# zhaoyuhsin/Edge-Guided-Near-Eye-Image-Analysis-for-Head-Mounted-Displays

Measured on AMD Instinct MI355X. Metric: eye-frames/sec (320x240): inference edge+seg (value), +fit, exact fp32, and train fwd+bwd at 1 MI355X, higher is better.
Workload: dtype f32 tensors; inference products split into f16 hi/lo pairs (3 f16 MFMAs per product, 22-bit significand), f32 accumulate (`exact_fp32`: every product on the f32 MFMA); `train`: bf16 storage, f32 accumulate, f32 master weights (and an f32-storage leg)

## Files before the change

edge-guided-near-eye-image-analysis-for-head-mounted-displays_amd/csrc/common.h:

```cpp
#pragma once
#include <hip/hip_runtime.h>
#include <cstdarg>
#include <cstdio>
#include <mutex>
#include <unordered_map>
#include "../../include/egne_hip.h"

static __device__ __attribute__((aligned(256), used)) float egne_zero_page[64] = {0};

typedef __bf16 egne_bf16;
typedef float egne_f32x4 __attribute__((ext_vector_type(4)));
typedef __bf16 egne_bf16x4 __attribute__((ext_vector_type(4)));
typedef __bf16 egne_bf16x8 __attribute__((ext_vector_type(8)));

__device__ __forceinline__ egne_f32x4 ld4(const float* p) { return *(const egne_f32x4*)p; }
__device__ __forceinline__ egne_f32x4 ld4(const egne_bf16* p) { return __builtin_convertvector(*(const egne_bf16x4*)p, egne_f32x4); }
__device__ __forceinline__ void st4(float* p, egne_f32x4 v) { *(egne_f32x4*)p = v; }
__device__ __forceinline__ void st4(egne_bf16* p, egne_f32x4 v) { *(egne_bf16x4*)p = __builtin_convertvector(v, egne_bf16x4); }
__device__ __forceinline__ float ld1(const float* p) { return *p; }
__device__ __forceinline__ float ld1(const egne_bf16* p) { return (float)*p; }
__device__ __forceinline__ void st1(float* p, float v) { *p = v; }
__device__ __forceinline__ void st1(egne_bf16* p, float v) { *p = (egne_bf16)v; }
template <typename T> struct egne_vt { static constexpr int N = 4; };
template <> struct egne_vt<egne_bf16> { static constexpr int N = 8; };
template <int N> struct egne_fv { float v[N]; };
__device__ __forceinline__ egne_fv<4> ldv(const float* p) {
  const egne_f32x4 t = *(const egne_f32x4*)p;
  return egne_fv<4>{{t[0], t[1], t[2], t[3]}};
}
__device__ __forceinline__ egne_fv<8> ldv(const egne_bf16* p) {
  typedef unsigned u4_ __attribute__((ext_vector_type(4)));
  const u4_ w = *(const u4_*)p;
  egne_fv<8> r;
#pragma unroll
  for (int i = 0; i < 4; ++i) {
    r.v[2 * i] = __builtin_bit_cast(float, w[i] << 16);
    r.v[2 * i + 1] = __builtin_bit_cast(float, w[i] & 0xffff0000u);
  }
  return r;
}
__device__ __forceinline__ void stv(float* p, const egne_fv<4>& a) { *(egne_f32x4*)p = egne_f32x4{a.v[0], a.v[1], a.v[2], a.v[3]}; }
__device__ __forceinline__ void stv(egne_bf16* p, const egne_fv<8>& a) {
  const egne_f32x4 lo = {a.v[0], a.v[1], a.v[2], a.v[3]}, hi = {a.v[4], a.v[5], a.v[6], a.v[7]};
  const egne_bf16x4 l = __builtin_convertvector(lo, egne_bf16x4), h = __builtin_convertvector(hi, egne_bf16x4);
  *(egne_bf16x8*)p = egne_bf16x8{l[0], l[1], l[2], l[3], h[0], h[1], h[2], h[3]};
}
typedef unsigned egne_u32x4 __attribute__((ext_vector_type(4)));
template <typename T> __device__ __forceinline__ egne_u32x4 ldraw(const T* p) { return *(const egne_u32x4*)p; }
__device__ __forceinline__ egne_fv<4> unpackv(const float*, egne_u32x4 w) {
  return egne_fv<4>{{__builtin_bit_cast(float, w[0]), __builtin_bit_cast(float, w[1]), __builtin_bit_cast(float, w[2]), __builtin_bit_cast(float, w[3])}};
}
__device__ __forceinline__ egne_fv<8> unpackv(const egne_bf16*, egne_u32x4 w) {
  egne_fv<8> r;
#pragma unroll
  for (int i = 0; i < 4; ++i) {
    r.v[2 * i] = __builtin_bit_cast(float, w[i] << 16);
    r.v[2 * i + 1] = __builtin_bit_cast(float, w[i] & 0xffff0000u);
  }
  return r;
}
template <int N> __device__ __forceinline__ egne_fv<N> ldf(const float* p) {
  egne_fv<N> r;
#pragma unroll
  for (int i = 0; i < N; i += 4) { const egne_f32x4 t = *(const egne_f32x4*)(p + i); r.v[i] = t[0]; r.v[i + 1] = t[1]; r.v[i + 2] = t[2]; r.v[i + 3] = t[3]; }
  return r;
}
template <int N> __device__ __forceinline__ egne_fv<N> fv_fill(float x) {
  egne_fv<N> r;
#pragma unroll
  for (int i = 0; i < N; ++i) r.v[i] = x;
  return r;
}
template <typename T> __device__ __forceinline__ const T* zero_page() { return (const T*)egne_zero_page; }

#ifdef EGNE_NO_OVF_CHECK
__device__ __forceinline__ bool egne_nonfinite(float) { return false; }
__device__ __forceinline__ bool egne_nonfinite64(double) { return false; }
#else
__device__ __forceinline__ bool egne_nonfinite(float v) { return __builtin_amdgcn_classf(v, 0x207); }
__device__ __forceinline__ bool egne_nonfinite64(double v) { return !__builtin_isfinite(v); }
#endif
__device__ __forceinline__ bool egne_ovf_row(int y, int H) { return y % 3 == 1 || y == H - 1; }
__device__ __forceinline__ void egne_ovf_commit(bool bad, unsigned* flag) {
  if (flag && bad) atomicOr(flag, 1u);
}

namespace egne {

char* err_buf();

inline int fail(int code, const char* fmt, ...) {
  va_list ap;
  va_start(ap, fmt);
  vsnprintf(err_buf(), 512, fmt, ap);
  va_end(ap);
  return code;
}

inline bool fp32_storage(const egne_conv_desc& d) {
  for (int i = 0; i < d.nseg && i < EGNE_MAXSEG; ++i)
    if (d.seg[i].presplit != 0) return false;
  return d.out_split == 0;
}

inline int check_launch(const char* what) {
  hipError_t e = hipGetLastError();
  if (e != hipSuccess) return fail(EGNE_ERR_LAUNCH, "%s: %s", what, hipGetErrorString(e));
  return EGNE_OK;
}

inline bool raise_lds(const void* kern, size_t bytes) {
  static std::mutex mu;
  static std::unordered_map<const void*, size_t> have;
  std::lock_guard<std::mutex> g(mu);
  auto it = have.find(kern);
  if (it != have.end() && it->second >= bytes) return true;
  if (hipFuncSetAttribute(kern, hipFuncAttributeMaxDynamicSharedMemorySize, (int)bytes) != hipSuccess) {
    (void)hipGetLastError();
    return false;
  }
  have[kern] = bytes;
  return true;
}

#define EGNE_REQUIRE(cond, ...) \
  do { if (!(cond)) return ::egne::fail(EGNE_ERR_ARG, __VA_ARGS__); } while (0)

bool halo3_supported(const egne_conv_desc& d);
int halo3_launch(const egne_conv_desc& d, hipStream_t st);

bool wgrad_halo_supported(const egne_conv_desc& d, long long gzs);
int wgrad_halo_splits(const egne_conv_desc& d);
int wgrad_halo_launch(const egne_conv_desc& d, const float* gz, long long gzs, int gzo, float* ws, hipStream_t st);
int wgrad_halo_f16_launch(const egne_conv_desc& d, const float* gz, long long gzs, int gzo, const unsigned* gz_dyn, float* ws, hipStream_t st);

bool wgrad3x3_bf16_supported(const egne_conv_desc& d, long long gzs);
int wgrad3x3_bf16_splits(const egne_conv_desc& d);
int wgrad3x3_bf16_launch(const egne_conv_desc& d, const egne_bf16* gz, long long gzs, int gzo, float* ws, hipStream_t st);
bool wgrad1x1_bf16_supported(const egne_conv_desc& d, long long gzs);
int wgrad1x1_bf16_splits(const egne_conv_desc& d);
int wgrad1x1_bf16_launch(const egne_conv_desc& d, const egne_bf16* gz, long long gzs, int gzo, float* ws, hipStream_t st);

int msdil_ps_launch(const egne_conv_desc& d, const void* fhi, const void* flo, float a_scale, float w_scale, const float* score_w,
                    const float* score_c, float* s0, float* s1, int accumulate, hipStream_t st);

bool msdil1_wanted(const egne_conv_desc& d);
int msdil1_launch(const egne_conv_desc& d, const void* fhi, float a_scale, float w_scale, const float* score_w, const float* score_c,
                  float* s0, float* s1, int accumulate, hipStream_t st);

inline int cdiv(long long a, long long b) { return (int)((a + b - 1) / b); }

}
```

edge-guided-near-eye-image-analysis-for-head-mounted-displays_amd/csrc/msblock_dil_ps_f16.hip:

```cpp
#include "common.h"
#include <type_traits>

typedef float f32x4 __attribute__((ext_vector_type(4)));
typedef _Float16 h8 __attribute__((ext_vector_type(8)));
typedef unsigned u32x4 __attribute__((ext_vector_type(4)));
typedef __attribute__((address_space(3))) void* lds_ptr;

namespace {
__device__ int g_pdbg = 0;
__device__ unsigned long long g_pstamps[256 * 8 * 4];

constexpr int TW = 32, TH = 8;
constexpr int D0 = 4, D1 = 8, D2 = 12, DMAX = 12;
constexpr int SWMAX = TW + 2 * DMAX, NPXMAX = TH * SWMAX;
constexpr int PLANE = NPXMAX * 32 + 32;
constexpr int BUFH = 2 * PLANE;
constexpr int WBUFH = 12 * 512;
constexpr int NS = 9;
constexpr unsigned OOB = 0x80000000u;

__device__ __forceinline__ __amdgpu_buffer_rsrc_t make_rsrc(const void* base, unsigned bytes) {
  return __builtin_amdgcn_make_buffer_rsrc(const_cast<void*>(base), 0, (int)bytes, 0x00020000);
}

__device__ __forceinline__ void lds_barrier() {
  asm volatile("s_waitcnt lgkmcnt(0)" ::: "memory");
  __builtin_amdgcn_s_barrier();
  asm volatile("" ::: "memory");
}

constexpr int dil_of(int g) { return g == 0 ? D0 : (g == 1 ? D1 : D2); }
constexpr int ni_of(int g) { return TH * (TW + 2 * dil_of(g)) * 8 / 512; }

template <bool XIN, int NP = 3>
__global__ __launch_bounds__(512)
void msdil_ps_kernel(const egne_conv_desc p, const _Float16* __restrict__ fhi, const _Float16* __restrict__ flo, float inv_a, float out_scale,
                     int tiles_x, int tiles_y, int ntiles, int cols, const float* __restrict__ score_w, const float* __restrict__ score_c,
                     float* __restrict__ s0, float* __restrict__ s1, int accumulate) {
  extern __shared__ __attribute__((aligned(16))) _Float16 ldsh[];
  _Float16* const lw = ldsh + 2 * BUFH;
  float* const lconst = (float*)(lw + 3 * WBUFH);
  int* const lrel = (int*)(lconst + 162);

  const int dbg = g_pdbg;
  unsigned long long t_work = 0, t_wait = 0, t_last = __builtin_amdgcn_s_memtime();
  auto stamp = [&](unsigned long long& accum) {
    if (dbg & 64) {
      asm volatile("s_waitcnt lgkmcnt(0)" ::: "memory");
      const unsigned long long t = __builtin_amdgcn_s_memtime();
      accum += t - t_last; t_last = t;
    }
  };
  const int tid = threadIdx.x, lane = tid & 63;
  const int wave = __builtin_amdgcn_readfirstlane(tid >> 6);
  const int l15 = lane & 15, kg = lane >> 4;
  const int H = p.H, W = p.W;
  const egne_seg sg = p.seg[0];

  const int per = gridDim.x >> 3;
  auto tile_at = [&](int i) { return (gridDim.x & 7) ? (int)blockIdx.x + i * (int)gridDim.x : ((i * 8 + ((int)blockIdx.x & 7)) * per + ((int)blockIdx.x >> 3)); };
  struct Tile { int b, y0, x0; };
  auto decode = [&](int t) {
    Tile r;
    const int ntx = cols == 0 ? tiles_x : (cols == 1 ? tiles_x - 2 : 2);
    const int tq = t % ntx; t /= ntx;
    const int tx = cols == 0 ? tq : (cols == 1 ? tq + 1 : tq * (tiles_x - 1));
    const int ty = t % tiles_y; t /= tiles_y;
    r.b = t; r.y0 = ty * TH; r.x0 = tx * TW;
    return r;
  };
  int nmine = 0;
  while (tile_at(nmine) < ntiles) ++nmine;
  if (tid < 160) {
    const int r = tid >> 5, c = tid & 31;
    lconst[tid] = r < 3 ? (p.bias ? p.bias[r * p.CoutP + c] : 0.f) : (score_w ? score_w[(r - 3) * 32 + c] : 0.f);
  } else if (tid < 162) {
    lconst[tid] = score_c ? score_c[tid - 160] : 0.f;
  }

  const int piece = tid & 7, pg = tid >> 3;
  constexpr int NI0 = ni_of(0), NI1 = ni_of(1), NI2 = ni_of(2);
  u32x4 st0[NI0], st1[NI1], st2[NI2];
  auto stbuf = [&](auto gc) -> u32x4* { constexpr int Gq = decltype(gc)::value; if constexpr (Gq == 0) return st0; else if constexpr (Gq == 1) return st1; else return st2; };
  constexpr int RB1 = NI0, RB2 = NI0 + NI1;
  if constexpr (XIN) {
    for (int e = tid; e < (NI0 + NI1 + NI2) * 64; e += 512) {
      const int row = e >> 6, pgq = e & 63;
      const int g = row < RB1 ? 0 : (row < RB2 ? 1 : 2), I = row - (g == 0 ? 0 : (g == 1 ? RB1 : RB2));
      const int d = g == 0 ? D0 : (g == 1 ? D1 : D2), SW = TW + 2 * d;
      const int px = pgq + 64 * I;
      const int rr = px / SW, cc = px - rr * SW;
      lrel[e] = ((rr * W + cc - d) * (int)sg.pix_stride + sg.ch_off) * 4;
    }
  }
  const int lofs = (piece >> 2) * PLANE + pg * 32 + (((piece & 3) ^ ((pg >> 1) & 3)) << 3);
  const unsigned wbytes = 3u * 9u * 2u * 1024u;
  const __amdgpu_buffer_rsrc_t rwh = make_rsrc(fhi, wbytes), rwl = make_rsrc(flo, wbytes);

  auto dma_weights = [&](auto sc) {
    constexpr int S = decltype(sc)::value, g = S % 3, ky = S / 3;
    char* wb = (char*)(lw + g * WBUFH);
#pragma unroll
    for (int t = 0; t < 2; ++t) {
      const int j = t == 0 ? wave : 8 + (wave & 3), f = j >> 1;
      const int o = ((g * 9 + ky * 3 + (f >> 1)) * 2 + (f & 1)) * 1024;
      __builtin_amdgcn_raw_ptr_buffer_load_lds((j & 1) ? rwl : rwh, (lds_ptr)(wb + j * 1024), 16, lane * 16, o, 0, 0);
    }
  };
  auto issue_strip = [&](const Tile& tl, bool on, auto sc) {
    constexpr int S = decltype(sc)::value, g = S % 3, ky = S / 3, d = dil_of(g), SW = TW + 2 * d;
    const __amdgpu_buffer_rsrc_t r = make_rsrc(sg.ptr + (long long)tl.b * H * W * sg.pix_stride, (unsigned)H * W * (unsigned)sg.pix_stride * 4u);
    int pq = pg;
    asm volatile("" : "+v"(pq));
#pragma unroll
    for (int I = 0; I < ni_of(g); ++I) {
      int off;
      if constexpr (XIN) {
        const int sbase = ((tl.y0 + (ky - 1) * d) * W + tl.x0) * (int)sg.pix_stride * 4 + piece * 16;
        off = lrel[((g == 0 ? 0 : (g == 1 ? RB1 : RB2)) + I) * 64 + pq] + sbase;
      } else {
        const int px = pq + 64 * I;
        const int rr = px / SW, cc = px - rr * SW;
        const int y = tl.y0 + (ky - 1) * d + rr, x = tl.x0 - d + cc;
        off = ((y * W + x) * (int)sg.pix_stride + sg.ch_off + piece * 4) * 4;
        off = ((unsigned)x < (unsigned)W && (unsigned)y < (unsigned)H) ? off : (int)OOB;
      }
      stbuf(std::integral_constant<int, g>{})[I] = __builtin_amdgcn_raw_buffer_load_b128(r, (on && !(dbg & 1) && (NP == 3 || piece < 4)) ? off : (int)OOB, 0, 0);
    }
  };
  auto write_strip = [&](int q, auto sc) {
    constexpr int S = decltype(sc)::value, g = S % 3;
    _Float16* buf = ldsh + (q & 1) * BUFH;
    if (!(dbg & 2)) {
#pragma unroll
      for (int I = 0; I < ni_of(g); ++I) *(u32x4*)&buf[lofs + 32 * 64 * I] = stbuf(std::integral_constant<int, g>{})[I];
    }
  };

  const int wl = (kg >> 1) * 1024 + ((kg & 1) * 32 + l15) * 8;
  f32x4 acc[3][2][2];
  h8 resh[2], resl[2];
  auto compute_strip = [&](int q, auto sc) {
    constexpr int S = decltype(sc)::value, g = S % 3, ky = S / 3, d = dil_of(g), SW = TW + 2 * d;
    const _Float16* Shi = ldsh + (q & 1) * BUFH;
    const _Float16* Slo = Shi + PLANE;
    const _Float16* wb = lw + g * WBUFH + wl;
    if constexpr (ky == 0) {
#pragma unroll
      for (int a = 0; a < 4; ++a) (&acc[g][0][0])[a] = (f32x4)(0.f);
    }
    h8 wh[2], wo[2], ah[2][2], al[2][2];
    auto fetch_w = [&](auto kc) {
      constexpr int KX = decltype(kc)::value;
#pragma unroll
      for (int nh = 0; nh < 2; ++nh) {
        wh[nh] = *(const h8*)&wb[KX * 2048 + nh * 128];
        if constexpr (NP == 3) wo[nh] = *(const h8*)&wb[KX * 2048 + 512 + nh * 128];
      }
    };
    auto fetch = [&](auto kc) {
      constexpr int KX = decltype(kc)::value, Bq = KX & 1;
#pragma unroll
      for (int ph = 0; ph < 2; ++ph) {
        const int qq = wave * SW + ph * 16 + l15 + KX * d;
        const int o = qq * 32 + ((kg ^ ((qq >> 1) & 3)) << 3);
        ah[Bq][ph] = *(const h8*)&Shi[o];
        if constexpr (NP == 3 || (S == 3 && KX == 1)) al[Bq][ph] = *(const h8*)&Slo[o];
      }
    };
    fetch(std::integral_constant<int, 0>{});
    [&]<int... Ks>(std::integer_sequence<int, Ks...>) {
      (([&] {
        constexpr int kx = Ks, Bq = kx & 1;
        fetch_w(std::integral_constant<int, kx>{});
        if constexpr (kx + 1 < 3) fetch(std::integral_constant<int, kx + 1>{});
        if constexpr (S == 3 && kx == 1) { resh[0] = ah[1][0]; resh[1] = ah[1][1]; resl[0] = al[1][0]; resl[1] = al[1][1]; }
        __builtin_amdgcn_sched_barrier(0);
        if constexpr (NP == 3) {
#pragma unroll
        for (int ph = 0; ph < 2; ++ph)
#pragma unroll
          for (int nh = 0; nh < 2; ++nh) acc[g][ph][nh] = __builtin_amdgcn_mfma_f32_16x16x32_f16(wh[nh], al[Bq][ph], acc[g][ph][nh], 0, 0, 0);
#pragma unroll
        for (int ph = 0; ph < 2; ++ph)
#pragma unroll
          for (int nh = 0; nh < 2; ++nh) acc[g][ph][nh] = __builtin_amdgcn_mfma_f32_16x16x32_f16(wo[nh], ah[Bq][ph], acc[g][ph][nh], 0, 0, 0);
        }
#pragma unroll
        for (int ph = 0; ph < 2; ++ph)
#pragma unroll
          for (int nh = 0; nh < 2; ++nh) acc[g][ph][nh] = __builtin_amdgcn_mfma_f32_16x16x32_f16(wh[nh], ah[Bq][ph], acc[g][ph][nh], 0, 0, 0);
        __builtin_amdgcn_sched_barrier(0);
      }()), ...);
    }(std::make_integer_sequence<int, 3>{});
  };

  const unsigned frame_out = (unsigned)H * W * (unsigned)p.out_pix_stride * 4u;
  float* sdst = nullptr;
  float sprev = 0.f;
  bool ovf_bad = false;
  auto score_prefetch = [&](const Tile& tl) {
    const int h = kg >> 1, y = tl.y0 + wave, x = tl.x0 + (kg & 1) * 16 + l15;
    sdst = (score_w && y < H && x < W) ? (h ? s1 : s0) + ((long long)tl.b * H + y) * W + x : nullptr;
    sprev = *(sdst ? (const volatile float*)sdst : (const volatile float*)p.residual);
  };
  auto epilogue = [&](const Tile& tl) {
    const int y = tl.y0 + wave;
    const __amdgpu_buffer_rsrc_t rout = make_rsrc(p.out ? p.out + (long long)tl.b * H * W * p.out_pix_stride : nullptr, p.out ? frame_out : 0u);
    f32x4 bq[3][2], cwq[2][2];
#pragma unroll
    for (int nh = 0; nh < 2; ++nh) {
      const int n = nh * 16 + 4 * kg;
#pragma unroll
      for (int g = 0; g < 3; ++g) bq[g][nh] = *(const f32x4*)&lconst[g * 32 + n];
#pragma unroll
      for (int h = 0; h < 2; ++h) cwq[h][nh] = *(const f32x4*)&lconst[(3 + h) * 32 + n];
    }
    float sc[2][2];
#pragma unroll
    for (int ph = 0; ph < 2; ++ph) {
      const int x = tl.x0 + ph * 16 + l15;
      const bool okp = y < H && x < W;
      const int pix = y * W + x;
      sc[0][ph] = sc[1][ph] = 0.f;
#pragma unroll
      for (int nh = 0; nh < 2; ++nh) {
        f32x4 v;
#pragma unroll
        for (int e = 0; e < 4; ++e) {
          const float o = ((float)resh[ph][nh * 4 + e] + (float)resl[ph][nh * 4 + e]) * inv_a;
          v[e] = fmaxf(acc[0][ph][nh][e] * out_scale + bq[0][nh][e], 0.f) + fmaxf(acc[1][ph][nh][e] * out_scale + bq[1][nh][e], 0.f) +
                 fmaxf(acc[2][ph][nh][e] * out_scale + bq[2][nh][e], 0.f) + o;
          sc[0][ph] += v[e] * cwq[0][nh][e];
          sc[1][ph] += v[e] * cwq[1][nh][e];
          if (nh == 0 && e == 0) ovf_bad |= egne_nonfinite(acc[0][ph][nh][e] + acc[1][ph][nh][e] + acc[2][ph][nh][e] + o);
        }
        if (p.out) {
          const int n = nh * 16 + 4 * kg;
          const int oo = (okp && n < p.Cout_store) ? (pix * (int)p.out_pix_stride + p.out_ch_off + n) * 4 : (int)OOB;
          __builtin_amdgcn_raw_buffer_store_b128(__builtin_bit_cast(u32x4, v), rout, oo, 0, 0);
        }
      }
    }
    if (score_w) {
#pragma unroll
      for (int h = 0; h < 2; ++h)
#pragma unroll
        for (int ph = 0; ph < 2; ++ph) {
          float t = sc[h][ph];
          t += __shfl_xor(t, 16);
          t += __shfl_xor(t, 32);
          sc[h][ph] = t;
        }
      const int h = kg >> 1, ph = kg & 1;
      const float v = h ? (ph ? sc[1][1] : sc[1][0]) : (ph ? sc[0][1] : sc[0][0]);
      if (sdst) *sdst = v + (accumulate ? sprev : lconst[160 + h]);
    }
  };

  __syncthreads();
  using I0 = std::integral_constant<int, 0>;
  using I1 = std::integral_constant<int, 1>;
  using I2 = std::integral_constant<int, 2>;
  if (nmine > 0) {
    const Tile t0 = decode(tile_at(0));
    dma_weights(I0{});
    dma_weights(I1{});
    issue_strip(t0, true, I0{});
    issue_strip(t0, true, I1{});
    issue_strip(t0, true, I2{});
    write_strip(0, I0{});
    issue_strip(t0, true, std::integral_constant<int, 3>{});
    asm volatile("s_waitcnt vmcnt(%0)" :: "n"(NI1 + NI2 + NI0) : "memory");
  }
  lds_barrier();
  for (int i = 0; i < nmine; ++i) {
    const Tile tl = decode(tile_at(i));
    const bool nx_on = i + 1 < nmine;
    const Tile nx = decode(tile_at(nx_on ? i + 1 : i));
    [&]<int... Ss>(std::integer_sequence<int, Ss...>) {
      (([&] {
        constexpr int S = Ss, S2 = (S + 2) % NS, S3 = (S + 3) % NS, S4 = (S + 4) % NS;
        const int q = 9 * i + S;
        dma_weights(std::integral_constant<int, S2>{});
        if constexpr (S == NS - 1) score_prefetch(tl);
        if constexpr (S + 1 < NS) write_strip(q + 1, std::integral_constant<int, S + 1>{});
        else if (nx_on) write_strip(q + 1, I0{});
        if constexpr (S + 4 < NS) issue_strip(tl, true, std::integral_constant<int, S4>{});
        else issue_strip(nx, nx_on, std::integral_constant<int, S4>{});
        compute_strip(q, std::integral_constant<int, S>{});
        if constexpr (S == NS - 1) epilogue(tl);
        stamp(t_work);
        asm volatile("s_waitcnt vmcnt(%0)" :: "n"(ni_of(S3 % 3) + 2 + ni_of(S4 % 3)) : "memory");
        lds_barrier();
        stamp(t_wait);
      }()), ...);
    }(std::make_integer_sequence<int, NS>{});
  }
  egne_ovf_commit(ovf_bad, p.ovf_flag);
  if ((dbg & 64) && lane == 0) {
    unsigned long long* o = g_pstamps + ((long long)blockIdx.x * 8 + wave) * 4;
    o[0] = t_work; o[1] = t_wait; o[2] = nmine; o[3] = 0;
  }
}

}

namespace egne {
int msdil_ps_launch(const egne_conv_desc& d, const void* fhi, const void* flo, float a_scale, float w_scale, const float* score_w,
                    const float* score_c, float* s0, float* s1, int accumulate, hipStream_t st) {
  if (msdil1_wanted(d)) return msdil1_launch(d, fhi, a_scale, w_scale, score_w, score_c, s0, s1, accumulate, st);
  const int tiles_x = (d.W + TW - 1) / TW, tiles_y = (d.H + TH - 1) / TH;
  const int ntiles = tiles_x * tiles_y * d.B;
  constexpr size_t lds = ((size_t)2 * BUFH + 2 * WBUFH) * sizeof(_Float16) + 162 * sizeof(float) + 18 * 64 * sizeof(int) + WBUFH * sizeof(_Float16);
  static_assert(lds <= 163840, "LDS budget");
  const float os = 1.0f / (a_scale * w_scale), inv_a = 1.0f / a_scale;
  const bool split = tiles_x > 2 && d.W >= TW * (tiles_x - 1) + 12;
  auto go = [&](auto npc) -> int {
    constexpr int NP = decltype(npc)::value;
    static bool once = hipFuncSetAttribute((const void*)msdil_ps_kernel<false, NP>, hipFuncAttributeMaxDynamicSharedMemorySize, (int)lds) == hipSuccess &&
                       hipFuncSetAttribute((const void*)msdil_ps_kernel<true, NP>, hipFuncAttributeMaxDynamicSharedMemorySize, (int)lds) == hipSuccess;
    if (!once) return egne::fail(EGNE_ERR_LAUNCH, "msblock_dil (split-pair input): cannot raise the dynamic LDS limit to %zu", lds);
    if (split) {
      const int nt_in = (tiles_x - 2) * tiles_y * d.B, nt_b = 2 * tiles_y * d.B;
      hipLaunchKernelGGL((msdil_ps_kernel<true, NP>), dim3(nt_in < 256 ? nt_in : 256), dim3(512), lds, st, d, (const _Float16*)fhi, (const _Float16*)flo,
                         inv_a, os, tiles_x, tiles_y, nt_in, 1, score_w, score_c, s0, s1, accumulate);
      static const bool only_interior = getenv("EGNE_MSDIL_ONLY_INTERIOR") != nullptr;
      if (!only_interior) hipLaunchKernelGGL((msdil_ps_kernel<false, NP>), dim3(nt_b < 256 ? nt_b : 256), dim3(512), lds, st, d, (const _Float16*)fhi,
                                             (const _Float16*)flo, inv_a, os, tiles_x, tiles_y, nt_b, 2, score_w, score_c, s0, s1, accumulate);
    } else {
      hipLaunchKernelGGL((msdil_ps_kernel<false, NP>), dim3(ntiles < 256 ? ntiles : 256), dim3(512), lds, st, d, (const _Float16*)fhi, (const _Float16*)flo,
                         inv_a, os, tiles_x, tiles_y, ntiles, 0, score_w, score_c, s0, s1, accumulate);
    }
    return EGNE_OK;
  };
  const int rc = d.f16_products == 1 ? go(std::integral_constant<int, 1>{}) : go(std::integral_constant<int, 3>{});
  if (rc != EGNE_OK) return rc;
  return egne::check_launch("egne_msblock_dil_f16_fwd (split-pair input)");
}
}

extern "C" int egne_msdil_ps_debug(int dbg, void* out_stamps) {
  if (hipMemcpyToSymbol(HIP_SYMBOL(g_pdbg), &dbg, sizeof(int)) != hipSuccess) return -2;
  if (out_stamps && hipMemcpyFromSymbol(out_stamps, HIP_SYMBOL(g_pstamps), sizeof(unsigned long long) * 256 * 8 * 4) != hipSuccess) return -2;
  return 0;
}
```

Measured before the change: 2120.

## Add phase-plane ring kernel for dilated msblock split-pair forward

Adds a new kernel for the dilated multi-scale block (dilations 4/8/12) that splits the image into 16 stride-4 phase planes, so each dilation becomes a small-halo (±3) conv on a decimated grid. Row groups are streamed through a three-slot LDS ring with weight DMA pipelined across the nine taps, and work is split into column and row segments picked by a simple cost model. The goal is to shrink halo loads and LDS footprint compared with the wide-halo tile kernel. The cost is strided gathers per phase and extra code-path complexity.

```diff
diff --git a/edge-guided-near-eye-image-analysis-for-head-mounted-displays_amd/csrc/common.h b/edge-guided-near-eye-image-analysis-for-head-mounted-displays_amd/csrc/common.h
--- a/edge-guided-near-eye-image-analysis-for-head-mounted-displays_amd/csrc/common.h
+++ b/edge-guided-near-eye-image-analysis-for-head-mounted-displays_amd/csrc/common.h
@@ -148,6 +148,10 @@
 int msdil1_launch(const egne_conv_desc& d, const void* fhi, float a_scale, float w_scale, const float* score_w, const float* score_c,
                   float* s0, float* s1, int accumulate, hipStream_t st);
 
+bool msdil3_wanted(const egne_conv_desc& d);
+int msdil3_launch(const egne_conv_desc& d, const void* fhi, const void* flo, float a_scale, float w_scale, const float* score_w,
+                  const float* score_c, float* s0, float* s1, int accumulate, hipStream_t st);
+
 inline int cdiv(long long a, long long b) { return (int)((a + b - 1) / b); }
 
 }
diff --git a/edge-guided-near-eye-image-analysis-for-head-mounted-displays_amd/csrc/msblock_dil3_f16.hip b/edge-guided-near-eye-image-analysis-for-head-mounted-displays_amd/csrc/msblock_dil3_f16.hip
--- /dev/null
+++ b/edge-guided-near-eye-image-analysis-for-head-mounted-displays_amd/csrc/msblock_dil3_f16.hip
@@ -0,0 +1,321 @@
+#include "common.h"
+#include <cstdlib>
+#include <type_traits>
+#include <utility>
+
+typedef float f32x4 __attribute__((ext_vector_type(4)));
+typedef _Float16 h8 __attribute__((ext_vector_type(8)));
+typedef unsigned u32x4 __attribute__((ext_vector_type(4)));
+typedef __attribute__((address_space(3))) void* lds_ptr;
+
+namespace {
+
+constexpr int TW = 32, TH = 8, HALO = 3;
+constexpr int RPX = TW + 2 * HALO;
+constexpr int GPX = TH * RPX, GROUPB = GPX * 64;
+constexpr int NGRP = 3, RROWS = NGRP * TH;
+constexpr int PLANEB = NGRP * GROUPB;
+constexpr int OFF_LO = PLANEB + 64;
+constexpr int RINGB = 2 * PLANEB + 128;
+constexpr int WBUFB = 12 * 1024;
+constexpr int OFF_W = RINGB, OFF_DUMMY = OFF_W + 3 * WBUFB, OFF_CONST = OFF_DUMMY + 1024;
+constexpr int LDS_BYTES = OFF_CONST + 164 * 4;
+constexpr int GK = GPX / 16;
+constexpr int GI = 2 * GK, GJ = 5;
+constexpr int NS = 9;
+constexpr unsigned OOB = 0x80000000u;
+static_assert(GPX % 16 == 0 && ((GPX >> 1) & 3) == 0, "a group holds whole instructions and leaves the swizzle key alone");
+static_assert(GJ * 8 >= GI && LDS_BYTES <= 163840, "LDS budget");
+
+__device__ __forceinline__ __amdgpu_buffer_rsrc_t make_rsrc(const void* base, unsigned bytes) {
+  return __builtin_amdgcn_make_buffer_rsrc(const_cast<void*>(base), 0, (int)bytes, 0x00020000);
+}
+
+__device__ __forceinline__ void lds_barrier() {
+  asm volatile("s_waitcnt lgkmcnt(0)" ::: "memory");
+  __builtin_amdgcn_s_barrier();
+  asm volatile("" ::: "memory");
+}
+
+__global__ __launch_bounds__(512)
+void msdil3_kernel(const egne_conv_desc p, const _Float16* __restrict__ fhi, const _Float16* __restrict__ flo, float inv_a, float out_scale,
+                   int ncols, int nseg, int seg_rows, int nitems, const float* __restrict__ score_w, const float* __restrict__ score_c,
+                   float* __restrict__ s0, float* __restrict__ s1, int accumulate) {
+  extern __shared__ __attribute__((aligned(1024))) char lds[];
+  float* const lconst = (float*)(lds + OFF_CONST);
+  const int tid = threadIdx.x, lane = tid & 63;
+  const int wave = __builtin_amdgcn_readfirstlane(tid >> 6);
+  const int l15 = lane & 15, kg = lane >> 4;
+  const int H = p.H, W = p.W, B = p.B;
+  const egne_seg sg = p.seg[0];
+
+  if (tid < 160) {
+    const int r = tid >> 5, c = tid & 31;
+    lconst[tid] = r < 3 ? (p.bias ? p.bias[r * p.CoutP + c] : 0.f) : (score_w ? score_w[(r - 3) * 32 + c] : 0.f);
+  } else if (tid < 162) {
+    lconst[tid] = score_c ? score_c[tid - 160] : 0.f;
+  }
+
+  const unsigned wbytes = 3u * 9u * 2u * 1024u;
+  const __amdgpu_buffer_rsrc_t rwh = make_rsrc(fhi, wbytes), rwl = make_rsrc(flo, wbytes);
+  auto dma_weights = [&](auto sc) {
+    constexpr int S = decltype(sc)::value, g = S % 3, ky = S / 3;
+    char* wb = lds + OFF_W + g * WBUFB;
+#pragma unroll
+    for (int t = 0; t < 2; ++t) {
+      const int j = t == 0 ? wave : 8 + (wave & 3), f = j >> 1;
+      const int o = ((g * 9 + ky * 3 + (f >> 1)) * 2 + (f & 1)) * 1024;
+      __builtin_amdgcn_raw_ptr_buffer_load_lds((j & 1) ? rwl : rwh, (lds_ptr)(wb + j * 1024), 16, lane * 16, o, 0, 0);
+    }
+  };
+
+  int rel[GJ], rr[GJ], cc[GJ];
+#pragma unroll
+  for (int j = 0; j < GJ; ++j) {
+    const int k = wave * GJ + j, plane = k >= GK, kk = k - plane * GK;
+    const int slot = 16 * kk + (lane >> 2);
+    const int r = slot / RPX, c = slot - r * RPX;
+    rr[j] = k < GI ? r : -100000;
+    cc[j] = c - HALO;
+    rel[j] = ((r * W + c - HALO) * 4 * (int)sg.pix_stride + sg.ch_off) * 4 + plane * 64 + (((lane & 3) ^ ((slot >> 1) & 3)) << 4);
+  }
+  const int wl = ((kg >> 1) * 1024 + ((kg & 1) * 32 + l15) * 8) * 2;
+
+  const unsigned frame_in = (unsigned)H * W * (unsigned)sg.pix_stride * 4u;
+  const unsigned frame_out = (unsigned)H * W * (unsigned)p.out_pix_stride * 4u;
+  bool ovf_bad = false;
+
+  using I0 = std::integral_constant<int, 0>;
+  using I1 = std::integral_constant<int, 1>;
+  dma_weights(I0{});
+  dma_weights(I1{});
+
+  for (int it = (int)blockIdx.x; it < nitems; it += (int)gridDim.x) {
+    const int sgi = it % nseg, r1 = it / nseg, phase = r1 & 15, r2 = r1 >> 4, b = r2 % B, cx = r2 / B;
+    const int py = phase >> 2, px = phase & 3;
+    const int Hp = (H - py + 3) >> 2, Wp = (W - px + 3) >> 2;
+    const int C0 = cx * TW, ys = sgi * seg_rows;
+    const int ye = ys + seg_rows < Hp ? ys + seg_rows : Hp;
+    if (ys >= ye || C0 >= Wp) continue;
+    const int nst = (ye - ys + TH - 1) / TH;
+    const bool two = Wp - C0 > 16;
+    const __amdgpu_buffer_rsrc_t rin = make_rsrc(sg.ptr + (long long)b * H * W * sg.pix_stride, frame_in);
+    const __amdgpu_buffer_rsrc_t rout = make_rsrc(p.out ? p.out + (long long)b * H * W * p.out_pix_stride : nullptr, p.out ? frame_out : 0u);
+    auto issue_group = [&](int Rg, int slot, bool on) {
+      const int sbase = ((4 * Rg + py) * W + 4 * C0 + px) * (int)sg.pix_stride * 4;
+#pragma unroll
+      for (int j = 0; j < GJ; ++j) {
+        const bool ok = on && (unsigned)(Rg + rr[j]) < (unsigned)Hp && (unsigned)(C0 + cc[j]) < (unsigned)Wp;
+        const int k = wave * GJ + j;
+        char* dst = k < GI ? lds + (k >= GK ? OFF_LO - GK * 1024 : 0) + slot * GROUPB + k * 1024 : lds + OFF_DUMMY;
+        __builtin_amdgcn_raw_ptr_buffer_load_lds(rin, (lds_ptr)dst, 16, ok ? rel[j] + sbase : (int)OOB, 0, 0, 0);
+      }
+    };
+    issue_group(ys - HALO, 0, true);
+    issue_group(ys - HALO + TH, 1, true);
+    asm volatile("s_waitcnt vmcnt(0)" ::: "memory");
+    lds_barrier();
+
+    int t3 = 0;
+    for (int t = 0; t < nst; ++t) {
+      const int y0 = ys + TH * t;
+      int qrow[7];
+#pragma unroll
+      for (int j = 0; j < 7; ++j) {
+        int rho = TH * t3 + wave + j;
+        rho = rho >= RROWS ? rho - RROWS : rho;
+        qrow[j] = rho * RPX + l15;
+      }
+      const int gnext = t3 == 0 ? 2 : t3 - 1;
+      const bool more = t + 1 < nst;
+
+      auto step = [&](auto nphc) {
+        constexpr int NPH = decltype(nphc)::value;
+        f32x4 acc[3][2][2];
+        h8 resh[2], resl[2];
+        float* sdst = nullptr;
+        float sprev = 0.f;
+
+        auto compute = [&](auto sc) {
+          constexpr int S = decltype(sc)::value, g = S % 3, ky = S / 3, dd = g + 1, jr = 3 + (ky - 1) * dd;
+          const char* wb = lds + OFF_W + g * WBUFB + wl;
+          if constexpr (ky == 0) {
+#pragma unroll
+            for (int a = 0; a < 4; ++a) (&acc[g][0][0])[a] = (f32x4)(0.f);
+          }
+          h8 wh[2], wo[2], ah[2][2], al[2][2];
+          auto fetch_w = [&](auto kc) {
+            constexpr int KX = decltype(kc)::value;
+#pragma unroll
+            for (int nh = 0; nh < 2; ++nh) {
+              wh[nh] = *(const h8*)(wb + KX * 4096 + nh * 256);
+              wo[nh] = *(const h8*)(wb + KX * 4096 + 1024 + nh * 256);
+            }
+          };
+          auto fetch = [&](auto kc) {
+            constexpr int KX = decltype(kc)::value, Bq = KX & 1;
+#pragma unroll
+            for (int ph = 0; ph < NPH; ++ph) {
+              const int qq = qrow[jr] + (HALO + (KX - 1) * dd + 16 * ph);
+              const int o = qq * 64 + ((kg ^ ((qq >> 1) & 3)) << 4);
+              ah[Bq][ph] = *(const h8*)(lds + o);
+              al[Bq][ph] = *(const h8*)(lds + OFF_LO + o);
+            }
+          };
+          fetch(I0{});
+          [&]<int... Ks>(std::integer_sequence<int, Ks...>) {
+            (([&] {
+              constexpr int kx = Ks, Bq = kx & 1;
+              fetch_w(std::integral_constant<int, kx>{});
+              if constexpr (kx + 1 < 3) fetch(std::integral_constant<int, kx + 1>{});
+              if constexpr (S == 3 && kx == 1) {
+#pragma unroll
+                for (int ph = 0; ph < NPH; ++ph) { resh[ph] = ah[1][ph]; resl[ph] = al[1][ph]; }
+              }
+              __builtin_amdgcn_sched_barrier(0);
+#pragma unroll
+              for (int ph = 0; ph < NPH; ++ph)
+#pragma unroll
+                for (int nh = 0; nh < 2; ++nh) acc[g][ph][nh] = __builtin_amdgcn_mfma_f32_16x16x32_f16(wh[nh], al[Bq][ph], acc[g][ph][nh], 0, 0, 0);
+#pragma unroll
+              for (int ph = 0; ph < NPH; ++ph)
+#pragma unroll
+                for (int nh = 0; nh < 2; ++nh) acc[g][ph][nh] = __builtin_amdgcn_mfma_f32_16x16x32_f16(wo[nh], ah[Bq][ph], acc[g][ph][nh], 0, 0, 0);
+#pragma unroll
+              for (int ph = 0; ph < NPH; ++ph)
+#pragma unroll
+                for (int nh = 0; nh < 2; ++nh) acc[g][ph][nh] = __builtin_amdgcn_mfma_f32_16x16x32_f16(wh[nh], ah[Bq][ph], acc[g][ph][nh], 0, 0, 0);
+              __builtin_amdgcn_sched_barrier(0);
+            }()), ...);
+          }(std::make_integer_sequence<int, 3>{});
+        };
+
+        auto epilogue = [&] {
+          const int R = y0 + wave, y = 4 * R + py;
+          f32x4 bq[3][2], cwq[2][2];
+#pragma unroll
+          for (int nh = 0; nh < 2; ++nh) {
+            const int n = nh * 16 + 4 * kg;
+#pragma unroll
+            for (int g = 0; g < 3; ++g) bq[g][nh] = *(const f32x4*)&lconst[g * 32 + n];
+#pragma unroll
+            for (int h = 0; h < 2; ++h) cwq[h][nh] = *(const f32x4*)&lconst[(3 + h) * 32 + n];
+          }
+          float sc[2][2];
+          sc[0][1] = sc[1][1] = 0.f;
+#pragma unroll
+          for (int ph = 0; ph < NPH; ++ph) {
+            const int Cq = C0 + ph * 16 + l15, x = 4 * Cq + px;
+            const bool okp = R < Hp && Cq < Wp;
+            const int pix = y * W + x;
+            sc[0][ph] = sc[1][ph] = 0.f;
+#pragma unroll
+            for (int nh = 0; nh < 2; ++nh) {
+              f32x4 v;
+#pragma unroll
+              for (int e = 0; e < 4; ++e) {
+                const float o = ((float)resh[ph][nh * 4 + e] + (float)resl[ph][nh * 4 + e]) * inv_a;
+                v[e] = fmaxf(acc[0][ph][nh][e] * out_scale + bq[0][nh][e], 0.f) + fmaxf(acc[1][ph][nh][e] * out_scale + bq[1][nh][e], 0.f) +
+                       fmaxf(acc[2][ph][nh][e] * out_scale + bq[2][nh][e], 0.f) + o;
+                sc[0][ph] += v[e] * cwq[0][nh][e];
+                sc[1][ph] += v[e] * cwq[1][nh][e];
+                if (nh == 0 && e == 0) ovf_bad |= egne_nonfinite(acc[0][ph][nh][e] + acc[1][ph][nh][e] + acc[2][ph][nh][e] + o);
+              }
+              if (p.out) {
+                const int n = nh * 16 + 4 * kg;
+                const int oo = (okp && n < p.Cout_store) ? (pix * (int)p.out_pix_stride + p.out_ch_off + n) * 4 : (int)OOB;
+                __builtin_amdgcn_raw_buffer_store_b128(__builtin_bit_cast(u32x4, v), rout, oo, 0, 0);
+              }
+            }
+          }
+          if (score_w) {
+#pragma unroll
+            for (int h = 0; h < 2; ++h)
+#pragma unroll
+              for (int ph = 0; ph < NPH; ++ph) {
+                float tt = sc[h][ph];
+                tt += __shfl_xor(tt, 16);
+                tt += __shfl_xor(tt, 32);
+                sc[h][ph] = tt;
+              }
+            const int h = kg >> 1, ph = kg & 1;
+            const float v = h ? (ph ? sc[1][1] : sc[1][0]) : (ph ? sc[0][1] : sc[0][0]);
+            if (sdst) *sdst = v + (accumulate ? sprev : lconst[160 + h]);
+          }
+        };
+
+        [&]<int... Ss>(std::integer_sequence<int, Ss...>) {
+          (([&] {
+            constexpr int S = Ss, S2 = (S + 2) % NS;
+            dma_weights(std::integral_constant<int, S2>{});
+            if constexpr (S == 0) issue_group(y0 + 2 * TH - HALO, gnext, more);
+            if constexpr (S == NS - 1) {
+              const int h = kg >> 1, R = y0 + wave, Cq = C0 + (kg & 1) * 16 + l15;
+              sdst = (score_w && R < Hp && Cq < Wp) ? (h ? s1 : s0) + ((long long)b * H + 4 * R + py) * W + 4 * Cq + px : nullptr;
+              sprev = *(sdst ? (const volatile float*)sdst : (const volatile float*)p.residual);
+            }
+            compute(std::integral_constant<int, S>{});
+            if constexpr (S == NS - 1) {
+              asm volatile("s_waitcnt vmcnt(0)" ::: "memory");
+              epilogue();
+            } else if constexpr (S == 1) {
+              asm volatile("s_waitcnt vmcnt(%0)" :: "n"(GJ + 2) : "memory");
+            } else if constexpr (S > 1) {
+              asm volatile("s_waitcnt vmcnt(2)" ::: "memory");
+            }
+            lds_barrier();
+          }()), ...);
+        }(std::make_integer_sequence<int, NS>{});
+      };
+      if (two) step(std::integral_constant<int, 2>{});
+      else step(I1{});
+      t3 = t3 == 2 ? 0 : t3 + 1;
+    }
+  }
+  asm volatile("s_waitcnt vmcnt(0)" ::: "memory");
+  egne_ovf_commit(ovf_bad, p.ovf_flag);
+}
+
+}
+
+namespace egne {
+
+bool msdil3_wanted(const egne_conv_desc& d) {
+  const char* e = getenv("EGNE_MSDIL3");
+  return !(e && atoi(e) == 0) && d.f16_products != 1 && d.seg[0].presplit == 1 && d.W >= 64 && d.H >= 48;
+}
+
+void msdil3_items(int B, int H, int W, int force, int* ncols, int* nseg, int* seg_rows, long long* nitems) {
+  const int Hp = (H + 3) / 4, Wp = (W + 3) / 4;
+  *ncols = (Wp + TW - 1) / TW;
+  int best = 1;
+  double best_t = 1e30;
+  for (int ns = 1; ns <= 4; ++ns) {
+    const int rows = ((Hp + ns - 1) / ns + TH - 1) / TH * TH;
+    if (ns > 1 && rows * (ns - 1) >= Hp) continue;
+    const long long items = (long long)B * 16 * *ncols * ns;
+    const double t = (double)((items + 255) / 256) * (rows / TH + 1.0);
+    if (force == ns) { best = ns; break; }
+    if (t < best_t) { best_t = t; best = ns; }
+  }
+  *nseg = best;
+  *seg_rows = ((Hp + best - 1) / best + TH - 1) / TH * TH;
+  *nitems = (long long)B * 16 * *ncols * best;
+}
+
+int msdil3_launch(const egne_conv_desc& d, const void* fhi, const void* flo, float a_scale, float w_scale, const float* score_w,
+                  const float* score_c, float* s0, float* s1, int accumulate, hipStream_t st) {
+  const char* e = getenv("EGNE_MSDIL3_SEGS");
+  int ncols, nseg, seg_rows;
+  long long nitems;
+  msdil3_items(d.B, d.H, d.W, e ? atoi(e) : 0, &ncols, &nseg, &seg_rows, &nitems);
+  if (nitems > 0x7fffffff - 256) return egne::fail(EGNE_ERR_ARG, "msblock_dil (phase-plane ring): %lld work items", nitems);
+  if (!egne::raise_lds((const void*)msdil3_kernel, LDS_BYTES))
+    return egne::fail(EGNE_ERR_LAUNCH, "msblock_dil (phase-plane ring): cannot raise the dynamic LDS limit to %d", LDS_BYTES);
+  const float os = 1.0f / (a_scale * w_scale), inv_a = 1.0f / a_scale;
+  hipLaunchKernelGGL(msdil3_kernel, dim3((unsigned)(nitems < 256 ? nitems : 256)), dim3(512), LDS_BYTES, st, d, (const _Float16*)fhi,
+                     (const _Float16*)flo, inv_a, os, ncols, nseg, seg_rows, (int)nitems, score_w, score_c, s0, s1, accumulate);
+  return egne::check_launch("egne_msblock_dil_f16_fwd (phase-plane ring)");
+}
+
+}
diff --git a/edge-guided-near-eye-image-analysis-for-head-mounted-displays_amd/csrc/msblock_dil_ps_f16.hip b/edge-guided-near-eye-image-analysis-for-head-mounted-displays_amd/csrc/msblock_dil_ps_f16.hip
--- a/edge-guided-near-eye-image-analysis-for-head-mounted-displays_amd/csrc/msblock_dil_ps_f16.hip
+++ b/edge-guided-near-eye-image-analysis-for-head-mounted-displays_amd/csrc/msblock_dil_ps_f16.hip
@@ -310,6 +310,7 @@
 int msdil_ps_launch(const egne_conv_desc& d, const void* fhi, const void* flo, float a_scale, float w_scale, const float* score_w,
                     const float* score_c, float* s0, float* s1, int accumulate, hipStream_t st) {
   if (msdil1_wanted(d)) return msdil1_launch(d, fhi, a_scale, w_scale, score_w, score_c, s0, s1, accumulate, st);
+  if (msdil3_wanted(d)) return msdil3_launch(d, fhi, flo, a_scale, w_scale, score_w, score_c, s0, s1, accumulate, st);
   const int tiles_x = (d.W + TW - 1) / TW, tiles_y = (d.H + TH - 1) / TH;
   const int ntiles = tiles_x * tiles_y * d.B;
   constexpr size_t lds = ((size_t)2 * BUFH + 2 * WBUFH) * sizeof(_Float16) + 162 * sizeof(float) + 18 * 64 * sizeof(int) + WBUFH * sizeof(_Float16);
```

New measurement: 2160 (median of 6 runs). 1.02x the previous value.
